# lucidrains/vector-quantize-pytorch

Measured on NVIDIA H100. Metric: vectors quantized/sec at dim=256, codebook=1024; indices bit-exact vs ref, higher is better.
Workload: dtype bf16

## Files before the change

### include/vqb200.h

```cpp
#ifndef VQB200_H
#define VQB200_H

#include <stddef.h>
#include <stdint.h>

#ifdef __cplusplus
extern "C" {
#endif

#define VQB_VERSION 100

#define VQB_DTYPE_F32 0
#define VQB_DTYPE_BF16 1

#define VQB_METRIC_EUCLID 0
#define VQB_METRIC_COSINE 1

#define VQB_OK 0
#define VQB_E_INVALID -1
#define VQB_E_UNSUPPORTED -2
#define VQB_E_ALIGN -3
#define VQB_E_NO_DEVICE -4
#define VQB_E_DRIVER -5
#define VQB_E_WORKSPACE -6
// ... 18 lines not shown
  void* resid_out;
  void* qsum;
  float* stats_cnt;
  float* stats_sum;
  int dtype;
  void* planes_out;
} vqb_fused_outputs;

int vqb_version(void);
const char* vqb_strerror(int code);

int vqb_padded_codes(int K);

int vqb_codebook_prepare(const float* embed, int K, int D, int metric, void* planes, void* bext, float* bias,
                         float* cnorm2, float* cmax, void* stream);

int vqb_input_prepare(const void* x, int dtype, int64_t N, int D, int metric, void* x_eff, void* a_planes,
                      int n_planes, void* stream);

int vqb_assign(const void* a_planes, int n_a, int64_t N, int D, const void* b_planes, const void* bext,
               const float* cmax, int K, float margin_rel, int n_passes, int32_t* idx, vqb_flag_entry* flagged,
               int32_t* flag_count, float* dbg_best, const vqb_fused_outputs* fused , void* stream);

int vqb_assign_ex(const void* a_planes, int n_a, int64_t N, int D, const void* b_planes, const void* bext,
                  const float* cmax, int K, float margin_rel, int n_passes, int32_t* idx, vqb_flag_entry* flagged,
                  int32_t* flag_count, float* dbg_best, const vqb_fused_outputs* fused, int metric, const float* cnorm2,
                  void* stream);

int vqb_debug_set_profile_buffer(void* device_buffer);
int vqb_debug_active(void);
int vqb_debug_set_mode(int mode);
int vqb_debug_graph_stats(long long* out4);
int vqb_debug_assign_plan(int n_a, int D, int n_passes, int* out6);
int vqb_debug_stats_plan(int64_t N, int K, int sms, int* out3);

int vqb_fix_flagged(const void* x_eff, int dtype, int64_t N, int D, const float* embed, const float* cnorm2, int K,
                    int metric, vqb_flag_entry* flagged, const int32_t* flag_count, int32_t* idx,
                    const vqb_fused_outputs* fused , void* stream);

int vqb_gather(const void* x_eff, int dtype, int64_t N, int D, const float* embed, const int32_t* idx, void* q_out,
               int64_t* idx64_out, int64_t idx_stride, double* loss_sum, const void* x_raw, void* resid_out, void* qsum,
               void* stream);

int vqb_loss_finalize(const double* loss_sum, int64_t numel, int dtype, float weight, float* loss_out, void* stream);

int64_t vqb_stats_offset(int K);
int64_t vqb_stats_floats(int K, int D);
size_t vqb_ema_stats_workspace(int64_t N, int K);
int vqb_ema_stats(const void* x_eff, int dtype, int64_t N, int D, const int32_t* idx, int K, float* stats,
                  void* workspace, size_t workspace_bytes, void* stream);

int vqb_ema_apply(float* cluster_size, float* embed_avg, float* embed, const float* stats, int K, int D, double decay,
                  double eps, int metric, int do_lerp, int do_normalise, void* planes, void* bext, float* bias,
                  float* cnorm2, float* cmax, float* scratch, void* stream);

int vqb_ema_apply_weighted(float* cluster_size, float* embed_avg, float* embed, const float* stats, int K, int D,
                           double decay, double eps, int metric, int do_lerp, int do_normalise, const float* code_weight,
                           void* planes, void* bext, float* bias, float* cnorm2, float* cmax, float* scratch, void* stream);

int vqb_peer_barrier(void* const* peer_flags_host, int rank, int world, uint32_t* epoch_dev, void* stream);
int vqb_ema_apply_peers(float* cluster_size, float* embed_avg, float* embed, const void* const* peer_stats_host, int world,
                        int64_t slice_offset, int K, int D, double decay, double eps, int metric, int do_normalise,
                        const float* code_weight, void* planes, void* bext, float* bias, float* cnorm2, float* cmax,
                        float* scratch, void* stream);

typedef struct vqb_vq_forward_args {
// ... 125 lines not shown
```

### vector_quantize_pytorch_b200/_C.py

```python
import ctypes
import os

from . import build as _build

_c = ctypes
_i32, _i64, _f32, _f64, _vp, _sz = _c.c_int, _c.c_int64, _c.c_float, _c.c_double, _c.c_void_p, _c.c_size_t

DTYPE_F32, DTYPE_BF16 = 0, 1
METRIC_EUCLID, METRIC_COSINE = 0, 1

class FusedOutputs(ctypes.Structure):
    _fields_ = [("x_eff", _vp), ("embed", _vp), ("q_out", _vp), ("idx64_out", _vp), ("idx_stride", _i64),
                ("loss_sum", _vp), ("x_raw", _vp), ("resid_out", _vp), ("qsum", _vp), ("stats_cnt", _vp), ("stats_sum", _vp),
                ("dtype", _i32), ("planes_out", _vp)]


class VQForwardArgs(ctypes.Structure):
    _fields_ = [("x", _vp), ("dtype", _i32), ("metric", _i32), ("N", _i64), ("D", _i32), ("K", _i32),
                ("already_normalised", _i32), ("cluster_size", _vp), ("embed_avg", _vp), ("embed", _vp),
                ("planes", _vp), ("bext", _vp), ("bias", _vp), ("cnorm2", _vp), ("cmax", _vp), ("scratch", _vp),
                ("q_out", _vp), ("idx64_out", _vp), ("idx_stride", _i64), ("loss_out", _vp), ("loss_weight", _f32),
                ("resid_out", _vp), ("qsum", _vp), ("idx32", _vp), ("update", _i32), ("stats_mode", _i32), ("stats_accumulate", _i32), ("do_normalise", _i32),
                ("decay", _f64), ("eps", _f64), ("stats", _vp), ("margin_rel", _f32), ("workspace", _vp),
                ("workspace_bytes", _sz), ("ev_search_begin", _vp), ("ev_search_end", _vp),
# ... 35 lines not shown
                ("bar", RvqBarArgs), ("emap", RvqEmaPeersArgs), ("simvq", RvqSimvqArgs)]


RVQ_STAGE, RVQ_EMA, RVQ_ACCUMULATE, RVQ_BARRIER, RVQ_EMA_PEERS, RVQ_SIMVQ_TAIL = 0, 1, 2, 3, 4, 5

SIGNATURES = {
    "vqb_version": (_i32, []),
    "vqb_strerror": (_c.c_char_p, [_i32]),
    "vqb_padded_codes": (_i32, [_i32]),
    "vqb_codebook_prepare": (_i32, [_vp, _i32, _i32, _i32, _vp, _vp, _vp, _vp, _vp, _vp]),
    "vqb_input_prepare": (_i32, [_vp, _i32, _i64, _i32, _i32, _vp, _vp, _i32, _vp]),
    "vqb_assign": (_i32, [_vp, _i32, _i64, _i32, _vp, _vp, _vp, _i32, _f32, _i32, _vp, _vp, _vp, _vp, _vp, _vp]),
    "vqb_assign_ex": (_i32, [_vp, _i32, _i64, _i32, _vp, _vp, _vp, _i32, _f32, _i32, _vp, _vp, _vp, _vp, _vp, _i32, _vp, _vp]),
    "vqb_fix_flagged": (_i32, [_vp, _i32, _i64, _i32, _vp, _vp, _i32, _i32, _vp, _vp, _vp, _vp, _vp]),
    "vqb_gather": (_i32, [_vp, _i32, _i64, _i32, _vp, _vp, _vp, _vp, _i64, _vp, _vp, _vp, _vp, _vp]),
    "vqb_loss_finalize": (_i32, [_vp, _i64, _i32, _f32, _vp, _vp]),
    "vqb_stats_offset": (_i64, [_i32]),
    "vqb_stats_floats": (_i64, [_i32, _i32]),
    "vqb_ema_stats_workspace": (_sz, [_i64, _i32]),
    "vqb_ema_stats": (_i32, [_vp, _i32, _i64, _i32, _vp, _i32, _vp, _vp, _sz, _vp]),
    "vqb_ema_apply": (_i32, [_vp, _vp, _vp, _vp, _i32, _i32, _f64, _f64, _i32, _i32, _i32, _vp, _vp, _vp, _vp, _vp, _vp, _vp]),
    "vqb_rotate": (_i32, [_vp, _vp, _vp, _i64, _i32, _i32, _vp, _vp]),
    "vqb_diveq": (_i32, [_vp, _vp, _vp, _vp, _i64, _i32, _i32, _f32, _vp, _vp, _vp]),
    "vqb_peer_barrier": (_i32, [_vp, _i32, _i32, _vp, _vp]),
    "vqb_ema_apply_peers": (_i32, [_vp, _vp, _vp, _vp, _i32, _i64, _i32, _i32, _f64, _f64, _i32, _i32, _vp, _vp, _vp, _vp, _vp, _vp, _vp, _vp]),
    "vqb_ema_apply_weighted": (_i32, [_vp, _vp, _vp, _vp, _i32, _i32, _f64, _f64, _i32, _i32, _i32, _vp, _vp, _vp, _vp, _vp, _vp, _vp, _vp]),
    "vqb_vq_forward_workspace": (_sz, [_i64, _i32, _i32, _i32, _i32, _i32]),
    "vqb_vq_forward": (_i32, [_vp, _vp]),
    "vqb_debug_set_profile_buffer": (_i32, [_vp]),
    "vqb_debug_set_mode": (_i32, [_i32]),
    "vqb_debug_active": (_i32, []),
    "vqb_debug_graph_stats": (_i32, [_vp]),
    "vqb_debug_assign_plan": (_i32, [_i32, _i32, _i32, _vp]),
    "vqb_debug_stats_plan": (_i32, [_i64, _i32, _i32, _vp]),
    "vqb_decode": (_i32, [_vp, _i64, _i32, _i32, _i32, _vp, _i64, _vp, _i32, _vp]),
    "vqb_rvq_accumulate": (_i32, [_vp, _i64, _i32, _i32, _i32, _vp, _i64, _vp, _i32, _vp]),
    "vqb_debug_gather_sum_plan": (_i32, [_i32, _i32, _i32, _i32, _i64, _i32, _vp]),
    "vqb_rvq_forward": (_i32, [_vp, _i32, _vp]),
    "vqb_rsimvq_tail": (_i32, [_vp, _vp, _vp, _i64, _i32, _i32, _vp, _vp, _i32, _vp, _i64, _vp, _vp, _f32, _f32, _vp]),
    "vqb_rsimvq_backward": (_i32, [_vp, _vp, _i32, _i32, _vp, _i64, _i32, _i32, _i32, _vp, _vp, _vp, _vp]),
    "vqb_fsq_forward": (_i32, [_vp, _i32, _i32, _i64, _i32, _i32, _i32, _i32, _i32, _i32, _vp, _vp, _vp, _vp, _vp, _i32, _i64, _i64,
                               _i64, _vp]),
    "vqb_fsq_backward": (_i32, [_vp, _i32, _i32, _i64, _i32, _i32, _i32, _i32, _i32, _i32, _vp, _vp, _vp, _vp, _vp, _vp]),
    "vqb_fsq_decode": (_i32, [_vp, _i32, _i64, _i64, _i64, _i64, _i32, _i32, _i32, _i32, _i32, _vp, _vp, _vp, _vp, _vp, _vp]),
    "vqb_lfq_forward": (_i32, [_vp, _i32, _i64, _i32, _i32, _i32, _i32, _i32, _i32, _i32, _vp, _vp, _vp, _i64, _i64, _i64, _vp, _vp,
                               _vp, _i32, _vp]),
    "vqb_lfq_forward_blocks": (_i32, [_i64, _i32]),
    "vqb_lfq_entropy": (_i32, [_vp, _i64, _i32, _i32, _i32, _vp, _i64, _i64, _vp, _f32, _i32, _vp, _vp, _vp]),
    "vqb_lfq_entropy_tiles": (_i32, [_i32]),
    "vqb_lfq_entropy_backward": (_i32, [_vp, _i64, _i32, _i32, _i32, _vp, _i64, _i64, _vp, _f32, _vp, _vp, _i32, _vp, _vp, _vp]),
    "vqb_lfq_backward": (_i32, [_vp, _i32, _i64, _i32, _i32, _i32, _i32, _i32, _i32, _i32, _vp, _vp, _vp, _vp, _vp, _vp, _vp]),
    "vqb_lfq_decode": (_i32, [_vp, _i32, _i64, _i64, _i64, _i64, _i32, _i32, _i32, _vp, _vp, _vp, _vp]),
    "vqb_fsp_blocks": (_i32, [_i64]),
    "vqb_fsp_forward": (_i32, [_vp, _i32, _i64, _i32, _i32, _i32, _vp, _f32, _vp, _vp, _f32, _f32, _f32, _vp, _vp, _vp, _vp, _i32,
                               _vp]),
    "vqb_fsp_stats": (_i32, [_vp, _i32, _i64, _i32, _vp, _vp, _i32, _vp, _vp, _vp, _vp]),
    "vqb_fsp_backward": (_i32, [_vp, _i32, _i64, _i32, _i32, _i32, _vp, _i32, _vp, _vp, _vp, _vp, _vp, _vp]),
    "vqb_fsp_decode": (_i32, [_vp, _i32, _i64, _i32, _i32, _i32, _vp, _f32, _f32, _vp, _vp, _vp]),
    "vqb_binmap_hot": (_i32, [_vp, _vp, _i64, _i32, _vp, _vp]),
    "vqb_binmap_backward_plan": (_i32, [_i64, _i32, _i32, _vp]),
    "vqb_binmap_backward": (_i32, [_vp, _i64, _i32, _vp, _i64, _i64, _i32, _vp, _vp, _vp]),
}


def _load():
    path = os.environ.get("VQB200_LIB")
# ... 27 lines not shown
```

### vector_quantize_pytorch_b200/csrc/ptx.cuh

```cuda
#pragma once
#include <cuda.h>
#include <cuda_runtime.h>
#include <stdint.h>

namespace vqb {

__device__ __forceinline__ uint32_t smem_u32(const void* p) {
  return static_cast<uint32_t>(__cvta_generic_to_shared(p));
}

__device__ __forceinline__ void mbar_init(uint32_t bar, uint32_t count) {
  asm volatile("mbarrier.init.shared::cta.b64 [%0], %1;" ::"r"(bar), "r"(count));
}
__device__ __forceinline__ void fence_barrier_init() {
  asm volatile("fence.mbarrier_init.release.cluster;" ::: "memory");
}
__device__ __forceinline__ void mbar_arrive(uint32_t bar) {
  asm volatile("mbarrier.arrive.shared::cta.b64 _, [%0];" ::"r"(bar) : "memory");
}
__device__ __forceinline__ void mbar_arrive_expect_tx(uint32_t bar, uint32_t bytes) {
  asm volatile("mbarrier.arrive.expect_tx.shared::cta.b64 _, [%0], %1;" ::"r"(bar), "r"(bytes) : "memory");
}
__device__ __forceinline__ bool mbar_try_wait(uint32_t bar, uint32_t parity) {
  uint32_t ok;
  asm volatile(
      "{\n"
      ".reg .pred p;\n"
      "mbarrier.try_wait.parity.shared::cta.b64 p, [%1], %2;\n"
      "selp.u32 %0, 1, 0, p;\n"
      "}\n"
      : "=r"(ok)
      : "r"(bar), "r"(parity)
      : "memory");
  return ok != 0;
}

#ifndef VQB_WAIT_TIMEOUT_CYCLES
#define VQB_WAIT_TIMEOUT_CYCLES (8000000000ll)
#endif
__device__ __forceinline__ void mbar_wait(uint32_t bar, uint32_t parity) {
  if (mbar_try_wait(bar, parity)) return;
  const long long t0 = clock64();
  while (!mbar_try_wait(bar, parity)) {
    if (clock64() - t0 > VQB_WAIT_TIMEOUT_CYCLES) __trap();
  }
}

__device__ __forceinline__ void tma_prefetch_desc(const CUtensorMap* m) {
  asm volatile("prefetch.tensormap [%0];" ::"l"(reinterpret_cast<uint64_t>(m)) : "memory");
}
__device__ __forceinline__ void tma_load_3d(uint32_t dst, const CUtensorMap* m, uint32_t bar, int c0, int c1, int c2) {
  asm volatile(
      "cp.async.bulk.tensor.3d.shared::cluster.global.tile.mbarrier::complete_tx::bytes [%0], [%1, {%3, %4, %5}], [%2];"
      ::"r"(dst), "l"(reinterpret_cast<uint64_t>(m)), "r"(bar), "r"(c0), "r"(c1), "r"(c2)
      : "memory");
}

__device__ __forceinline__ void tma_prefetch_l2_3d(const CUtensorMap* m, int c0, int c1, int c2) {
  asm volatile("cp.async.bulk.prefetch.tensor.3d.L2.global.tile [%0, {%1, %2, %3}];"
               ::"l"(reinterpret_cast<uint64_t>(m)), "r"(c0), "r"(c1), "r"(c2)
               : "memory");
}

__device__ __forceinline__ uint64_t wgmma_desc_sw128(uint32_t saddr) {
  uint64_t d = 0;
  d |= static_cast<uint64_t>((saddr >> 4) & 0x3FFF);
  d |= static_cast<uint64_t>(1) << 16;
  d |= static_cast<uint64_t>(1024 >> 4) << 32;
  d |= static_cast<uint64_t>(1) << 62;
  return d;
}

__device__ __forceinline__ uint64_t wgmma_desc_sw32(uint32_t saddr) {
  uint64_t d = 0;
  d |= static_cast<uint64_t>((saddr >> 4) & 0x3FFF);
  d |= static_cast<uint64_t>(1) << 16;
  d |= static_cast<uint64_t>(256 >> 4) << 32;
  d |= static_cast<uint64_t>(3) << 62;
  return d;
}

__device__ __forceinline__ void fence_proxy_async_shared() { asm volatile("fence.proxy.async.shared::cta;" ::: "memory"); }
__device__ __forceinline__ void wgmma_fence() { asm volatile("wgmma.fence.sync.aligned;" ::: "memory"); }
__device__ __forceinline__ void wgmma_commit() { asm volatile("wgmma.commit_group.sync.aligned;" ::: "memory"); }
template <int N>
__device__ __forceinline__ void wgmma_wait() { asm volatile("wgmma.wait_group.sync.aligned %0;" ::"n"(N) : "memory"); }

// ... 158 lines not shown
```

### vector_quantize_pytorch_b200/csrc/vq_assign.cu

```cuda
#include <type_traits>
#include "ptx.cuh"
#include "vqb_common.cuh"
#include "gather_row.cuh"
#include "epilogue.cuh"

#ifdef VQB_PROFILE
#define PROF_CLOCK() clock64()
#else
#define PROF_CLOCK() 0ll
#endif

namespace vqb {

constexpr int BM = 128;
constexpr int WM = 64;
constexpr int BN_STAGE = 128;
constexpr int BK = 64;
constexpr int A_SUB_BYTES = BM * BK * 2;
constexpr int B_SUB_BYTES = BN_STAGE * BK * 2;
constexpr int MAX_A_SUB = 8;
constexpr int MAX_STAGES = 8;
constexpr int NUM_CONSUMER_WARPS = 8;
constexpr int NUM_STORE_WARPS = 3;
constexpr int NUM_THREADS = 128 + NUM_CONSUMER_WARPS * 32;
constexpr int SMEM_CTRL_BYTES = 14336;
constexpr int SMEM_LIMIT = 232448;
constexpr int SEED_BYTES = BN_STAGE * 32;

struct AssignParams {
  int64_t N;
  int D, K, Kpad;
  int n_a, n_passes;
  int KB;
  int n_stages;
  int n_seed;
  int stream_a;
  const uint16_t* a_global;
  const uint16_t* bext;
  int num_row_tiles, num_code_steps;
  float margin_rel;
  const float* cmax;
  int32_t* idx;
  int32_t* idx_prov;
  int32_t* hist;
  int hist_shift;
  vqb_flag_entry* flagged;
  int32_t* flag_count;
  float* dbg_best;
  const uint8_t* row_mask;
  long long* prof;
  FusedOut fo;
  int copy_mode;
  int resid_mode;
  int metric;
  const uint16_t* b_hi;
  const float* cnorm2;
  uint32_t tagmask, mul1, mulm1;
// ... 54 lines not shown

template <int TAIL, int WN>
__global__ void __launch_bounds__(NUM_THREADS, 1)
vq_assign_kernel(const __grid_constant__ CUtensorMap tmA, const __grid_constant__ CUtensorMap tmB,
                 const __grid_constant__ CUtensorMap tmS, const AssignParams p) {
  static_assert(WN == 128 || WN == 256, "code step width");
  constexpr int SPAN = WN / BN_STAGE;
  constexpr uint32_t STEP_SEED_BYTES = SPAN * SEED_BYTES;
  extern __shared__ __align__(1024) uint8_t smem[];
  Ctrl* ctrl = reinterpret_cast<Ctrl*>(smem);
  const uint32_t smem_base = smem_u32(smem);
  const uint32_t a_base = (smem_base + SMEM_CTRL_BYTES + 1023u) & ~1023u;
  const bool stream_a = WN == 128 && p.stream_a;
  const int n_sub = stream_a ? 0 : p.n_a * p.KB;
  const uint32_t b_base = a_base + n_sub * A_SUB_BYTES;
  const uint32_t a_stage_bytes = stream_a ? A_SUB_BYTES : 0;
  const uint32_t stage_stride = a_stage_bytes + SPAN * B_SUB_BYTES;
  const int n_ring = p.n_stages / SPAN;
  const uint32_t seed_base = b_base + n_ring * stage_stride;

  const int warp = threadIdx.x >> 5;
  const int lane = threadIdx.x & 31;

  if (threadIdx.x == 0) {
    tma_prefetch_desc(&tmA);
    tma_prefetch_desc(&tmB);
    tma_prefetch_desc(&tmS);
    for (int s = 0; s < n_sub; ++s) {
      mbar_init(smem_u32(&ctrl->a_full[s]), 1);
      mbar_init(smem_u32(&ctrl->a_empty[s]), NUM_CONSUMER_WARPS);
    }
    for (int s = 0; s < n_ring; ++s) {
      mbar_init(smem_u32(&ctrl->b_full[s]), 1);
      mbar_init(smem_u32(&ctrl->b_empty[s]), NUM_CONSUMER_WARPS);
    }
    for (int s = 0; s < 2; ++s) {
      mbar_init(smem_u32(&ctrl->g_full[s]), NUM_CONSUMER_WARPS);
      mbar_init(smem_u32(&ctrl->g_empty[s]), NUM_STORE_WARPS);
    }
    fence_barrier_init();
  }
  if constexpr (WN == 256) {
    for (int i = threadIdx.x; i < WM * 16 / 2; i += NUM_THREADS) StepLocals<256>::bias_ones()[i] = 0x3F803F80u;
    fence_proxy_async_shared();
  }
  __syncthreads();

  if (warp == 0) {
    if (lane == 0) {
      long long w_empty = 0, w_aempty = 0;
      const long long pstart = PROF_CLOCK();
      int stage = 0, gstep = 0;
      uint32_t ph = 0;
      for (int t = 0, tile = static_cast<int>(blockIdx.x); tile < p.num_row_tiles; ++t, tile += static_cast<int>(gridDim.x)) {
        const int row0 = tile * BM;
        if (!stream_a && tile + static_cast<int>(gridDim.x) < p.num_row_tiles) {
          for (int ap = 0; ap < p.n_a; ++ap)
            for (int kb = 0; kb < p.KB; ++kb) tma_prefetch_l2_3d(&tmA, kb * BK, row0 + static_cast<int>(gridDim.x) * BM, ap);
        }
        for (int ct = 0; ct < p.num_code_steps; ++ct, ++gstep) {
          for (int kb = 0; kb < p.KB; ++kb) {
            for (int ps = 0; ps < p.n_passes; ++ps) {
              const int bplane = (ps == 1) ? 1 : 0;
              const int aplane = (ps == 2) ? 1 : 0;
              if (!stream_a && ct == 0 && (ps == 0 || ps == 2)) {
                const int sub = aplane * p.KB + kb;
                { const long long c0 = PROF_CLOCK(); mbar_wait(smem_u32(&ctrl->a_empty[sub]), (t & 1) ^ 1); w_aempty += PROF_CLOCK() - c0; }
                mbar_arrive_expect_tx(smem_u32(&ctrl->a_full[sub]), A_SUB_BYTES);
                tma_load_3d(a_base + sub * A_SUB_BYTES, &tmA, smem_u32(&ctrl->a_full[sub]), kb * BK, row0, aplane);
              }
              { const long long c0 = PROF_CLOCK(); mbar_wait(smem_u32(&ctrl->b_empty[stage]), ph ^ 1); w_empty += PROF_CLOCK() - c0; }
              const bool seeds = kb == 0 && ps == 0;
              mbar_arrive_expect_tx(smem_u32(&ctrl->b_full[stage]), stage_stride + (seeds ? STEP_SEED_BYTES : 0));
              if (seeds)
                tma_load_3d(seed_base + (gstep % p.n_seed) * STEP_SEED_BYTES, &tmS, smem_u32(&ctrl->b_full[stage]), 0, ct * WN, 0);
              if (stream_a)
                tma_load_3d(b_base + stage * stage_stride, &tmA, smem_u32(&ctrl->b_full[stage]), kb * BK, row0, aplane);
              tma_load_3d(b_base + stage * stage_stride + a_stage_bytes, &tmB, smem_u32(&ctrl->b_full[stage]), kb * BK,
                          ct * WN, bplane);
              if (++stage == n_ring) { stage = 0; ph ^= 1; }
            }
          }
        }
      }
      if (p.prof) {
        p.prof[blockIdx.x * 16 + 0] = w_empty;
        p.prof[blockIdx.x * 16 + 1] = PROF_CLOCK() - pstart;
        p.prof[blockIdx.x * 16 + 6] = w_aempty;
      }
    }
  } else if (warp <= NUM_STORE_WARPS) {
    const int sw = warp - 1;
    float lsum = 0.f;
    for (int t = 0, tile = static_cast<int>(blockIdx.x); p.fo.enabled && tile < p.num_row_tiles; ++t, tile += static_cast<int>(gridDim.x)) {
      mbar_wait(smem_u32(&ctrl->g_full[t & 1]), (t >> 1) & 1);
      const int* gi = ctrl->gidx[t & 1];
      if (TAIL >= 1) {
        constexpr int CB = 4;
        const bool bf = p.fo.dtype == VQB_DTYPE_BF16;
        const int row_bytes = p.D * (bf ? 2 : 4);
        const uint8_t* src = bf ? reinterpret_cast<const uint8_t*>(p.b_hi) : reinterpret_cast<const uint8_t*>(p.fo.embed);
        const uint8_t* xin = static_cast<const uint8_t*>(p.fo.x_eff);
        uint8_t* dst = static_cast<uint8_t*>(TAIL == 2 ? p.fo.resid_out : p.fo.q_out);
        for (int r0 = sw * CB; r0 < BM; r0 += NUM_STORE_WARPS * CB) {
          int ks[CB];
          bool ex[CB];
#pragma unroll
          for (int b = 0; b < CB; ++b) {
            const int g = gi[r0 + b];
            ex[b] = g < -1;
            ks[b] = ex[b] ? -2 - g : g;
          }
          const int64_t row_base = static_cast<int64_t>(tile) * BM + r0;
          if (p.fo.idx64_out && lane < CB && ks[lane & (CB - 1)] >= 0) {
            int kk = 0;
#pragma unroll
            for (int b = 0; b < CB; ++b) kk = (lane == b) ? ks[b] : kk;
            p.fo.idx64_out[(row_base + lane) * p.fo.idx_stride] = kk;
          }
          if (dst || (ex[0] | ex[1] | ex[2] | ex[3])) {
            for (int off = lane * 16; off < row_bytes; off += 512) {
              uint4 v[CB];
#pragma unroll
              for (int b = 0; b < CB; ++b)
                if (ks[b] >= 0) v[b] = __ldg(reinterpret_cast<const uint4*>(src + static_cast<int64_t>(ks[b]) * row_bytes + off));
              if (TAIL == 1) {
#pragma unroll
// ... 43 lines not shown
          bool any = false;
#pragma unroll
          for (int b = 0; b < GB; ++b) {
            ks[b] = gi[r0 + b];
            rows[b] = ks[b] >= 0 ? static_cast<int64_t>(tile) * BM + r0 + b : -1;
            any |= ks[b] >= 0;
          }
          if (!any) continue;
          lsum += tail_rows<GB>(p.fo, rows, ks, p.D, lane);
        }
      }
      __syncwarp();
      if (lane == 0) mbar_arrive(smem_u32(&ctrl->g_empty[t & 1]));
    }
    if (p.fo.enabled && p.fo.loss_sum) {
      const double w = warp_sum(static_cast<double>(lsum));
      if (lane == 0) atomicAdd(p.fo.loss_sum, w);
    }
  } else {
    const int wg = (warp >> 2) - 1;
    const int q = lane & 3;
    const int rit0 = wg * WM + (warp & 3) * 16 + (lane >> 2);
    const int n_items = p.KB * p.n_passes;
    const uint32_t a_row_off = wg * WM * 128;
    const uint32_t bias_a = q == 0 ? 0x3F803F80u : (q == 1 ? 0x00003F80u : 0u);
    long long w_full = 0, w_afull = 0, w_gap = 0, gap0 = -1;
    const long long cstart = PROF_CLOCK();
    float acc[WN / 2];
    int stage = 0, gstep = 0;
    uint32_t ph = 0;
    StepLocals<WN> locals;
    auto release = [&](int st, int sub) {
      if (lane == 0) {
        mbar_arrive(smem_u32(&ctrl->b_empty[st]));
        if (sub >= 0) mbar_arrive(smem_u32(&ctrl->a_empty[sub]));
      }
    };
    auto row_norms = [&](int tile, float (&xlo)[2]) {
#pragma unroll
      for (int h = 0; h < 2; ++h) {
        const int64_t row = static_cast<int64_t>(tile) * BM + rit0 + 8 * h;
        float a = 0.f, alo = 0.f;
        if (row < p.N) {
          const uint16_t* hp = p.a_global + row * p.D;
          for (int c = q * 8; c < p.D; c += 32) {
            const uint4 u = __ldg(reinterpret_cast<const uint4*>(hp + c));
            uint4 l = make_uint4(0u, 0u, 0u, 0u);
            if (p.n_a == 2) l = __ldg(reinterpret_cast<const uint4*>(hp + p.N * p.D + c));
            const uint32_t w[4] = {u.x, u.y, u.z, u.w};
            const uint32_t wl[4] = {l.x, l.y, l.z, l.w};
#pragma unroll
            for (int e = 0; e < 4; ++e) {
              const float h0 = __uint_as_float(w[e] << 16), h1 = __uint_as_float(w[e] & 0xFFFF0000u);
              const float l0 = __uint_as_float(wl[e] << 16), l1 = __uint_as_float(wl[e] & 0xFFFF0000u);
              a = fmaf(h0 + l0, h0 + l0, a);
              a = fmaf(h1 + l1, h1 + l1, a);
              alo = fmaf(l0, l0, alo);
              alo = fmaf(l1, l1, alo);
            }
          }
        }
        a += __shfl_xor_sync(0xffffffffu, a, 1);
        a += __shfl_xor_sync(0xffffffffu, a, 2);
        alo += __shfl_xor_sync(0xffffffffu, alo, 1);
        alo += __shfl_xor_sync(0xffffffffu, alo, 2);
        if (q == 0) ctrl->x2[rit0 + 8 * h] = a;
        xlo[h] = alo;
      }
    };
    auto init_band = [&](auto (&sc)[2], float (&xlo)[2]) {
      const bool euclid = p.metric != VQB_METRIC_COSINE;
      const float cmax = __ldg(p.cmax + CMAX_NORM);
      const float cres = __ldg(p.cmax + CMAX_RES);
      const float caux = p.n_a == 2 ? 0x1.02p-8f * cmax + __ldg(p.cmax + CMAX_LO) : 0.f;
      __syncwarp();
#pragma unroll
      for (int h = 0; h < 2; ++h) {
        const float x2 = ctrl->x2[rit0 + 8 * h];
        const float xn = sqrtf(x2);
        const float xc = xn * cmax;
        xlo[h] = p.n_a == 2 ? sqrtf(xlo[h]) * 1.0001f : 0.f;
        sc[h].init(2.f * (xn * cres + xlo[h] * caux + p.margin_rel * xc + (euclid ? 0x1p-21f * cmax * cmax : 0.f)) +
                   0x1p-18f * (xc + (euclid ? 0.5f * cmax * cmax : 0.f)) +
                   (euclid ? 0x1p-22f * (x2 + cmax * cmax) + 1e-8f : 1e-30f));
      }
    };
    for (int t = 0, tile = static_cast<int>(blockIdx.x); tile < p.num_row_tiles; ++t, tile += static_cast<int>(gridDim.x)) {
      typename std::conditional<WN == 128, ScanReg, ScanState<16>>::type sc[2];
      ScanQueue<16> sq[2];

      float xlo[2] = {0.f, 0.f};
      for (int ct = 0; ct < p.num_code_steps; ++ct) {
        const bool last_ct = ct == p.num_code_steps - 1;
        if (WN == 256 && ct == 0) {
          row_norms(tile, xlo);
          init_band(sc, xlo);
        }
        if (gap0 >= 0) w_gap += PROF_CLOCK() - gap0;
        { const long long c0 = PROF_CLOCK(); mbar_wait(smem_u32(&ctrl->b_full[stage]), ph); w_full += PROF_CLOCK() - c0; }
        wgmma_fence();
        const uint64_t sd = wgmma_desc_sw32(seed_base + (gstep % p.n_seed) * STEP_SEED_BYTES);
        if constexpr (WN == 128) wgmma_m64n128k16_bf16_rs_set(acc, bias_a, sd);
        else wgmma_m64n256k16_bf16_ss_set(acc, wgmma_desc_sw32(smem_u32(StepLocals<256>::bias_ones())), sd);
        int kb = 0, ps = 0;
        int pend_stage = -1, pend_sub = -1;
        for (int i = 0; i < n_items; ++i) {
          const int aplane = (ps == 2) ? 1 : 0;
          const int sub = aplane * p.KB + kb;
          if (ct == 0 && !stream_a) { const long long c0 = PROF_CLOCK(); mbar_wait(smem_u32(&ctrl->a_full[sub]), t & 1); w_afull += PROF_CLOCK() - c0; }
          if (i > 0) { const long long c0 = PROF_CLOCK(); mbar_wait(smem_u32(&ctrl->b_full[stage]), ph); w_full += PROF_CLOCK() - c0; }
          const uint32_t st_addr = b_base + stage * stage_stride;
          const uint32_t a_addr = (stream_a ? st_addr : a_base + sub * A_SUB_BYTES) + a_row_off;
          const uint64_t ad = wgmma_desc_sw128(a_addr);
          const uint64_t bd = wgmma_desc_sw128(st_addr + a_stage_bytes);
          fence_regs(acc);
          wgmma_fence();
#pragma unroll
          for (int k = 0; k < 8; k += 2) {
            if constexpr (WN == 128) wgmma_m64n128k16_bf16(acc, ad + k, bd + k);
            else wgmma_m64n256k16_bf16(acc, ad + k, bd + k);
// ... 76 lines not shown
            p.idx[row] = i0;
            if (p.idx_prov) p.idx_prov[row] = (n < 2) ? i0 : -1;
            if (p.hist && n < 2) atomicAdd(p.hist + static_cast<size_t>(tile >> p.hist_shift) * p.K + i0, 1);
            if (p.dbg_best) p.dbg_best[row] = best;
            if (n >= 2) {
              const bool many = n > 3;
              const int s = many ? static_cast<int>(p.N) - 1 - atomicAdd(p.flag_count + 1, 1) : atomicAdd(p.flag_count, 1);
              vqb_flag_entry e;
              e.row = static_cast<int32_t>(row);
              e.cand0 = many ? 0 : i0;
              e.cand1 = many ? 0 : i1;
              e.cand2 = rr.i2;
              e.count = n;
              e.pad[0] = e.pad[1] = e.pad[2] = 0;
              p.flagged[s] = e;
            }
          }
        }
        __syncwarp();
      }
      if (p.fo.enabled && lane == 0) mbar_arrive(smem_u32(&ctrl->g_full[t & 1]));
    }
    if (TAIL >= 1 && p.fo.loss_sum) {
      const double w = warp_sum(static_cast<double>(locals.loss()));
      if (lane == 0) atomicAdd(p.fo.loss_sum, w);
    }
    if (p.prof && threadIdx.x == 128) {
      p.prof[blockIdx.x * 16 + 2] = w_full;
      p.prof[blockIdx.x * 16 + 3] = PROF_CLOCK() - cstart;
      p.prof[blockIdx.x * 16 + 4] = w_gap;
      p.prof[blockIdx.x * 16 + 5] = w_afull;
    }
  }
}

typedef CUresult (*PFN_encodeTiled)(CUtensorMap*, CUtensorMapDataType, cuuint32_t, void*, const cuuint64_t*,
                                    const cuuint64_t*, const cuuint32_t*, const cuuint32_t*, CUtensorMapInterleave,
                                    CUtensorMapSwizzle, CUtensorMapL2promotion, CUtensorMapFloatOOBfill);

static PFN_encodeTiled get_encode_fn() {
  static PFN_encodeTiled fn = nullptr;
  static bool tried = false;
  if (!tried) {
    tried = true;
    void* f = nullptr;
    cudaDriverEntryPointQueryResult qres;
    if (cudaGetDriverEntryPoint("cuTensorMapEncodeTiled", &f, cudaEnableDefault, &qres) == cudaSuccess &&
        qres == cudaDriverEntryPointSuccess)
      fn = reinterpret_cast<PFN_encodeTiled>(f);
  }
  return fn;
}

static int make_map(CUtensorMap* m, const void* base, int cols, int64_t rows, int planes, int box_cols, int box_rows,
                    CUtensorMapSwizzle swz) {
  PFN_encodeTiled enc = get_encode_fn();
  if (!enc) return VQB_E_DRIVER;
  cuuint64_t dims[3] = {static_cast<cuuint64_t>(cols), static_cast<cuuint64_t>(rows), static_cast<cuuint64_t>(planes)};
  cuuint64_t strides[2] = {static_cast<cuuint64_t>(cols) * 2, static_cast<cuuint64_t>(cols) * 2 * static_cast<cuuint64_t>(rows)};
  cuuint32_t box[3] = {static_cast<cuuint32_t>(box_cols), static_cast<cuuint32_t>(box_rows), 1};
  cuuint32_t estr[3] = {1, 1, 1};
  CUresult r = enc(m, CU_TENSOR_MAP_DATA_TYPE_BFLOAT16, 3, const_cast<void*>(base), dims, strides, box, estr,
                   CU_TENSOR_MAP_INTERLEAVE_NONE, swz, CU_TENSOR_MAP_L2_PROMOTION_L2_256B, CU_TENSOR_MAP_FLOAT_OOB_FILL_NONE);
  return r == CUDA_SUCCESS ? VQB_OK : VQB_E_DRIVER;
}

// ... 6 lines not shown
  if (n_passes == 0) n_passes = n_a + 1;
  if (n_passes != n_a + 1) return VQB_E_UNSUPPORTED;
  if (D % 8 != 0) return VQB_E_UNSUPPORTED;
  const int KB = (D + BK - 1) / BK;
  const int stream_a = n_a * KB > MAX_A_SUB ? 1 : 0;
  const int a_bytes = stream_a ? 0 : n_a * KB * A_SUB_BYTES;
  const int stage_bytes = B_SUB_BYTES + (stream_a ? A_SUB_BYTES : 0);
  const int fixed = SMEM_CTRL_BYTES + 1024  + a_bytes;
  const int n_items = KB * n_passes;
  int stages = MAX_STAGES;
  auto seed_slots = [&](int st) { return (st + n_items - 1) / n_items; };
  while (stages >= 2 && fixed + stages * stage_bytes + seed_slots(stages) * SEED_BYTES > SMEM_LIMIT) --stages;
  if (stages < 2) return VQB_E_UNSUPPORTED;
  pl->stream_a = stream_a;
  pl->n_stages = stages;
  pl->n_seed = seed_slots(stages);
  pl->n_items = n_items;
  pl->KB = KB;
  pl->smem_bytes = fixed + stages * stage_bytes + pl->n_seed * SEED_BYTES;
  return VQB_OK;
}

static bool wide_step(const AssignPlan& pl, int Kpad, int* n_seed, int* smem_bytes) {
  if (pl.stream_a || pl.n_stages % 2 != 0 || Kpad <= BN_STAGE) return false;
  const int ring = pl.n_stages / 2;
  const int seeds = (ring + pl.n_items - 1) / pl.n_items;
  const int bytes = pl.smem_bytes - pl.n_seed * SEED_BYTES + seeds * 2 * SEED_BYTES;
  if (bytes + WIDE_STATIC_SMEM > SMEM_LIMIT) return false;
  *n_seed = seeds;
  *smem_bytes = bytes;
  return true;
}

}

using namespace vqb;

extern "C" int vqb_debug_assign_plan(int n_a, int D, int n_passes, int* out6) {
  if (!out6) return VQB_E_INVALID;
  AssignPlan pl;
  const int rc = assign_plan(n_a, D, n_passes, &pl);
  if (rc) return rc;
  out6[0] = pl.stream_a; out6[1] = pl.n_stages; out6[2] = pl.n_seed;
  out6[3] = pl.n_items; out6[4] = pl.KB; out6[5] = pl.smem_bytes;
  return VQB_OK;
}

extern "C" int vqb_padded_codes(int K) {
  if (K <= 0) return 0;
  const int BN = code_tile(K);
  return (K + BN - 1) / BN * BN;
}

static long long* g_prof = nullptr;
static int g_dbg_mode = 0;
extern "C" int vqb_debug_set_mode(int mode) { g_dbg_mode = mode; return VQB_OK; }
extern "C" int vqb_debug_active(void) { return (g_prof != nullptr) || (g_dbg_mode != 0); }
extern "C" int vqb_debug_set_profile_buffer(void* buf) { g_prof = static_cast<long long*>(buf); return VQB_OK; }

extern "C" int vqb_assign(const void* a_planes, int n_a, int64_t N, int D, const void* b_planes, const void* bext,
                          const float* cmax, int K, float margin_rel, int n_passes, int32_t* idx,
                          vqb_flag_entry* flagged, int32_t* flag_count, float* dbg_best,
                          const vqb_fused_outputs* fused, void* stream) {
  return vqb_assign_ex(a_planes, n_a, N, D, b_planes, bext, cmax, K, margin_rel, n_passes, idx, flagged, flag_count,
                       dbg_best, fused, VQB_METRIC_EUCLID, nullptr, stream);
}

extern "C" int vqb_assign_ex(const void* a_planes, int n_a, int64_t N, int D, const void* b_planes, const void* bext,
                             const float* cmax, int K, float margin_rel, int n_passes, int32_t* idx,
                             vqb_flag_entry* flagged, int32_t* flag_count, float* dbg_best,
                             const vqb_fused_outputs* fused, int metric, const float* cnorm2, void* stream) {
  return vqb::assign_launch(a_planes, n_a, N, D, b_planes, bext, cmax, K, margin_rel, n_passes, idx, nullptr, nullptr, 0,
                            flagged, flag_count, dbg_best, fused, metric, cnorm2, stream);
}

int vqb::assign_launch(const void* a_planes, int n_a, int64_t N, int D, const void* b_planes, const void* bext,
                       const float* cmax, int K, float margin_rel, int n_passes, int32_t* idx, int32_t* idx_prov,
                       int32_t* hist, int hist_shift, vqb_flag_entry* flagged, int32_t* flag_count, float* dbg_best,
                       const vqb_fused_outputs* fused, int metric, const float* cnorm2, void* stream, const uint8_t* row_mask) {
  if (!a_planes || !b_planes || !bext || !cmax || !idx || !flagged || !flag_count) return VQB_E_INVALID;
  if (N <= 0 || K <= 0) return VQB_E_INVALID;
  AssignPlan plan;
  int rc = assign_plan(n_a, D, n_passes, &plan);
  if (rc) return rc;
// ... 5 lines not shown
  rc = make_fused(&p.fo, fused, D, N);
  if (rc) return rc;
  rc = check_device();
  if (rc) return rc;

  p.N = N; p.D = D; p.K = K;
  p.Kpad = vqb_padded_codes(K);
  p.n_a = n_a; p.n_passes = n_passes; p.KB = plan.KB;
  p.num_row_tiles = static_cast<int>((N + BM - 1) / BM);
  int smem_bytes = plan.smem_bytes;
  p.n_seed = plan.n_seed;
  const bool wide = wide_step(plan, p.Kpad, &p.n_seed, &smem_bytes);
  const int WN = wide ? 256 : 128;
  p.num_code_steps = (p.Kpad + WN - 1) / WN;
  p.margin_rel = margin_rel;
  p.cmax = cmax; p.idx = idx; p.idx_prov = idx_prov; p.hist = hist; p.hist_shift = hist_shift; p.flagged = flagged; p.flag_count = flag_count; p.dbg_best = dbg_best;
  p.row_mask = row_mask;
  p.prof = g_prof;
  p.tagmask = 0xFFFFFFF0u; p.mul1 = 1u; p.mulm1 = 0xFFFFFFFFu;
  p.metric = metric;
  p.cnorm2 = cnorm2;
  p.b_hi = static_cast<const uint16_t*>(b_planes);
  p.bext = static_cast<const uint16_t*>(bext);
  p.copy_mode = p.fo.enabled && !p.fo.resid_out && !(metric == VQB_METRIC_COSINE && p.fo.loss_sum && !cnorm2);
  p.resid_mode = p.fo.enabled && p.fo.resid_out && !p.fo.q_out &&
                 (!p.fo.x_raw || p.fo.x_raw == p.fo.x_eff) && !(metric == VQB_METRIC_COSINE && p.fo.loss_sum && !cnorm2);
  p.stream_a = plan.stream_a;
  p.a_global = static_cast<const uint16_t*>(a_planes);
  p.n_stages = plan.n_stages;

  CUtensorMap tmA, tmB, tmS;
  rc = make_map(&tmA, a_planes, D, N, n_a, BK, BM, CU_TENSOR_MAP_SWIZZLE_128B);
  if (rc) return rc;
  rc = make_map(&tmB, b_planes, D, p.Kpad, 2, BK, WN, CU_TENSOR_MAP_SWIZZLE_128B);
  if (rc) return rc;
  rc = make_map(&tmS, bext, 16, p.Kpad, 1, 16, WN, CU_TENSOR_MAP_SWIZZLE_32B);
  if (rc) return rc;

  static bool attr_set = false;
  if (!attr_set) {
    void (*const kernels[6])(CUtensorMap, CUtensorMap, CUtensorMap, AssignParams) = {
        vq_assign_kernel<0, 128>, vq_assign_kernel<1, 128>, vq_assign_kernel<2, 128>,
        vq_assign_kernel<0, 256>, vq_assign_kernel<1, 256>, vq_assign_kernel<2, 256>};
    for (int i = 0; i < 6; ++i) {
      const int dyn = i < 3 ? SMEM_LIMIT : SMEM_LIMIT - WIDE_STATIC_SMEM;
      const cudaError_t e = cudaFuncSetAttribute(kernels[i], cudaFuncAttributeMaxDynamicSharedMemorySize, dyn);
      if (e != cudaSuccess) return static_cast<int>(e);
    }
    attr_set = true;
  }
  const int grid = p.num_row_tiles < num_sms() ? p.num_row_tiles : num_sms();
  cudaStream_t s = static_cast<cudaStream_t>(stream);
  if (wide) {
    if (p.copy_mode) vq_assign_kernel<1, 256><<<grid, NUM_THREADS, smem_bytes, s>>>(tmA, tmB, tmS, p);
    else if (p.resid_mode) vq_assign_kernel<2, 256><<<grid, NUM_THREADS, smem_bytes, s>>>(tmA, tmB, tmS, p);
    else vq_assign_kernel<0, 256><<<grid, NUM_THREADS, smem_bytes, s>>>(tmA, tmB, tmS, p);
  } else {
    if (p.copy_mode) vq_assign_kernel<1, 128><<<grid, NUM_THREADS, smem_bytes, s>>>(tmA, tmB, tmS, p);
    else if (p.resid_mode) vq_assign_kernel<2, 128><<<grid, NUM_THREADS, smem_bytes, s>>>(tmA, tmB, tmS, p);
    else vq_assign_kernel<0, 128><<<grid, NUM_THREADS, smem_bytes, s>>>(tmA, tmB, tmS, p);
  }
  return static_cast<int>(cudaGetLastError());
}
```

Before: 389.1 million.

## Launch assign kernel as 2-CTA clusters with TMA multicast of codebook tiles

Launches the assign kernel in clusters of two CTAs. Each CTA loads half of every codebook (B) and seed tile and multicasts it to both CTAs, roughly halving L2-to-SMEM codebook traffic per CTA. Empty barriers now count arrivals from both CTAs, and cluster syncs are added at start and end. The grid is sized from cluster occupancy. In exchange the two CTAs are lockstepped, the row-tile loop bound is changed, and the odd CTA of the last pair may process an out-of-range tile.

```diff
diff --git a/include/vqb200.h b/include/vqb200.h
--- a/include/vqb200.h
+++ b/include/vqb200.h
@@ -74,6 +74,7 @@
 int vqb_debug_set_mode(int mode);
 int vqb_debug_graph_stats(long long* out4);
 int vqb_debug_assign_plan(int n_a, int D, int n_passes, int* out6);
+int vqb_debug_assign_grid(int n_a, int D, int K, int64_t N, int* out2);
 int vqb_debug_stats_plan(int64_t N, int K, int sms, int* out3);
 
 int vqb_fix_flagged(const void* x_eff, int dtype, int64_t N, int D, const float* embed, const float* cnorm2, int K,
diff --git a/vector_quantize_pytorch_b200/_C.py b/vector_quantize_pytorch_b200/_C.py
--- a/vector_quantize_pytorch_b200/_C.py
+++ b/vector_quantize_pytorch_b200/_C.py
@@ -91,6 +91,7 @@
     "vqb_debug_active": (_i32, []),
     "vqb_debug_graph_stats": (_i32, [_vp]),
     "vqb_debug_assign_plan": (_i32, [_i32, _i32, _i32, _vp]),
+    "vqb_debug_assign_grid": (_i32, [_i32, _i32, _i32, _i64, _vp]),
     "vqb_debug_stats_plan": (_i32, [_i64, _i32, _i32, _vp]),
     "vqb_decode": (_i32, [_vp, _i64, _i32, _i32, _i32, _vp, _i64, _vp, _i32, _vp]),
     "vqb_rvq_accumulate": (_i32, [_vp, _i64, _i32, _i32, _i32, _vp, _i64, _vp, _i32, _vp]),
diff --git a/vector_quantize_pytorch_b200/csrc/ptx.cuh b/vector_quantize_pytorch_b200/csrc/ptx.cuh
--- a/vector_quantize_pytorch_b200/csrc/ptx.cuh
+++ b/vector_quantize_pytorch_b200/csrc/ptx.cuh
@@ -46,6 +46,26 @@
   }
 }
 
+__device__ __forceinline__ uint32_t cluster_ctarank() {
+  uint32_t r;
+  asm volatile("mov.u32 %0, %%cluster_ctarank;" : "=r"(r));
+  return r;
+}
+__device__ __forceinline__ void mbar_arrive_pair(uint32_t bar) {
+  asm volatile(
+      "{\n"
+      ".reg .b32 r0, r1;\n"
+      "mapa.shared::cluster.u32 r0, %0, 0;\n"
+      "mapa.shared::cluster.u32 r1, %0, 1;\n"
+      "mbarrier.arrive.shared::cluster.b64 _, [r0];\n"
+      "mbarrier.arrive.shared::cluster.b64 _, [r1];\n"
+      "}\n" ::"r"(bar) : "memory");
+}
+__device__ __forceinline__ void cluster_sync() {
+  asm volatile("barrier.cluster.arrive.release;\n"
+               "barrier.cluster.wait.acquire;" ::: "memory");
+}
+
 __device__ __forceinline__ void tma_prefetch_desc(const CUtensorMap* m) {
   asm volatile("prefetch.tensormap [%0];" ::"l"(reinterpret_cast<uint64_t>(m)) : "memory");
 }
@@ -53,6 +73,15 @@
   asm volatile(
       "cp.async.bulk.tensor.3d.shared::cluster.global.tile.mbarrier::complete_tx::bytes [%0], [%1, {%3, %4, %5}], [%2];"
       ::"r"(dst), "l"(reinterpret_cast<uint64_t>(m)), "r"(bar), "r"(c0), "r"(c1), "r"(c2)
+      : "memory");
+}
+
+__device__ __forceinline__ void tma_load_3d_mc(uint32_t dst, const CUtensorMap* m, uint32_t bar, int c0, int c1, int c2,
+                                               uint16_t cta_mask) {
+  asm volatile(
+      "cp.async.bulk.tensor.3d.shared::cluster.global.tile.mbarrier::complete_tx::bytes.multicast::cluster"
+      " [%0], [%1, {%3, %4, %5}], [%2], %6;"
+      ::"r"(dst), "l"(reinterpret_cast<uint64_t>(m)), "r"(bar), "r"(c0), "r"(c1), "r"(c2), "h"(cta_mask)
       : "memory");
 }
 
diff --git a/vector_quantize_pytorch_b200/csrc/vq_assign.cu b/vector_quantize_pytorch_b200/csrc/vq_assign.cu
--- a/vector_quantize_pytorch_b200/csrc/vq_assign.cu
+++ b/vector_quantize_pytorch_b200/csrc/vq_assign.cu
@@ -23,6 +23,7 @@
 constexpr int NUM_CONSUMER_WARPS = 8;
 constexpr int NUM_STORE_WARPS = 3;
 constexpr int NUM_THREADS = 128 + NUM_CONSUMER_WARPS * 32;
+constexpr int PAIR = 2;
 constexpr int SMEM_CTRL_BYTES = 14336;
 constexpr int SMEM_LIMIT = 232448;
 constexpr int SEED_BYTES = BN_STAGE * 32;
@@ -143,7 +144,7 @@
     }
     for (int s = 0; s < n_ring; ++s) {
       mbar_init(smem_u32(&ctrl->b_full[s]), 1);
-      mbar_init(smem_u32(&ctrl->b_empty[s]), NUM_CONSUMER_WARPS);
+      mbar_init(smem_u32(&ctrl->b_empty[s]), PAIR * NUM_CONSUMER_WARPS);
     }
     for (int s = 0; s < 2; ++s) {
       mbar_init(smem_u32(&ctrl->g_full[s]), NUM_CONSUMER_WARPS);
@@ -155,7 +156,7 @@
     for (int i = threadIdx.x; i < WM * 16 / 2; i += NUM_THREADS) StepLocals<256>::bias_ones()[i] = 0x3F803F80u;
     fence_proxy_async_shared();
   }
-  __syncthreads();
+  cluster_sync();
 
   if (warp == 0) {
     if (lane == 0) {
@@ -163,7 +164,7 @@
       const long long pstart = PROF_CLOCK();
       int stage = 0, gstep = 0;
       uint32_t ph = 0;
-      for (int t = 0, tile = static_cast<int>(blockIdx.x); tile < p.num_row_tiles; ++t, tile += static_cast<int>(gridDim.x)) {
+      for (int t = 0, tile = static_cast<int>(blockIdx.x); (tile & ~1) < p.num_row_tiles; ++t, tile += static_cast<int>(gridDim.x)) {
         const int row0 = tile * BM;
         if (!stream_a && tile + static_cast<int>(gridDim.x) < p.num_row_tiles) {
           for (int ap = 0; ap < p.n_a; ++ap)
@@ -182,13 +183,16 @@
               }
               { const long long c0 = PROF_CLOCK(); mbar_wait(smem_u32(&ctrl->b_empty[stage]), ph ^ 1); w_empty += PROF_CLOCK() - c0; }
               const bool seeds = kb == 0 && ps == 0;
-              mbar_arrive_expect_tx(smem_u32(&ctrl->b_full[stage]), stage_stride + (seeds ? STEP_SEED_BYTES : 0));
+              const uint32_t full = smem_u32(&ctrl->b_full[stage]);
+              const int rank = static_cast<int>(cluster_ctarank());
+              mbar_arrive_expect_tx(full, stage_stride + (seeds ? STEP_SEED_BYTES : 0));
               if (seeds)
-                tma_load_3d(seed_base + (gstep % p.n_seed) * STEP_SEED_BYTES, &tmS, smem_u32(&ctrl->b_full[stage]), 0, ct * WN, 0);
+                tma_load_3d_mc(seed_base + (gstep % p.n_seed) * STEP_SEED_BYTES + rank * (WN / 2) * 32, &tmS, full, 0,
+                               ct * WN + rank * (WN / 2), 0, 0x3);
               if (stream_a)
-                tma_load_3d(b_base + stage * stage_stride, &tmA, smem_u32(&ctrl->b_full[stage]), kb * BK, row0, aplane);
-              tma_load_3d(b_base + stage * stage_stride + a_stage_bytes, &tmB, smem_u32(&ctrl->b_full[stage]), kb * BK,
-                          ct * WN, bplane);
+                tma_load_3d(b_base + stage * stage_stride, &tmA, full, kb * BK, row0, aplane);
+              tma_load_3d_mc(b_base + stage * stage_stride + a_stage_bytes + rank * (WN / 2) * 128, &tmB, full, kb * BK,
+                             ct * WN + rank * (WN / 2), bplane, 0x3);
               if (++stage == n_ring) { stage = 0; ph ^= 1; }
             }
           }
@@ -203,7 +207,7 @@
   } else if (warp <= NUM_STORE_WARPS) {
     const int sw = warp - 1;
     float lsum = 0.f;
-    for (int t = 0, tile = static_cast<int>(blockIdx.x); p.fo.enabled && tile < p.num_row_tiles; ++t, tile += static_cast<int>(gridDim.x)) {
+    for (int t = 0, tile = static_cast<int>(blockIdx.x); p.fo.enabled && (tile & ~1) < p.num_row_tiles; ++t, tile += static_cast<int>(gridDim.x)) {
       mbar_wait(smem_u32(&ctrl->g_full[t & 1]), (t >> 1) & 1);
       const int* gi = ctrl->gidx[t & 1];
       if (TAIL >= 1) {
@@ -313,7 +317,7 @@
     StepLocals<WN> locals;
     auto release = [&](int st, int sub) {
       if (lane == 0) {
-        mbar_arrive(smem_u32(&ctrl->b_empty[st]));
+        mbar_arrive_pair(smem_u32(&ctrl->b_empty[st]));
         if (sub >= 0) mbar_arrive(smem_u32(&ctrl->a_empty[sub]));
       }
     };
@@ -366,7 +370,7 @@
                    (euclid ? 0x1p-22f * (x2 + cmax * cmax) + 1e-8f : 1e-30f));
       }
     };
-    for (int t = 0, tile = static_cast<int>(blockIdx.x); tile < p.num_row_tiles; ++t, tile += static_cast<int>(gridDim.x)) {
+    for (int t = 0, tile = static_cast<int>(blockIdx.x); (tile & ~1) < p.num_row_tiles; ++t, tile += static_cast<int>(gridDim.x)) {
       typename std::conditional<WN == 128, ScanReg, ScanState<16>>::type sc[2];
       ScanQueue<16> sq[2];
 
@@ -509,6 +513,7 @@
       p.prof[blockIdx.x * 16 + 5] = w_afull;
     }
   }
+  cluster_sync();
 }
 
 typedef CUresult (*PFN_encodeTiled)(CUtensorMap*, CUtensorMapDataType, cuuint32_t, void*, const cuuint64_t*,
@@ -581,6 +586,47 @@
   return true;
 }
 
+typedef void (*AssignKernel)(CUtensorMap, CUtensorMap, CUtensorMap, AssignParams);
+static const AssignKernel kAssignKernels[6] = {
+    vq_assign_kernel<0, 128>, vq_assign_kernel<1, 128>, vq_assign_kernel<2, 128>,
+    vq_assign_kernel<0, 256>, vq_assign_kernel<1, 256>, vq_assign_kernel<2, 256>};
+
+static int resident_pairs(int ki, int smem_bytes, int* pairs) {
+  static bool attr_set = false;
+  if (!attr_set) {
+    for (int i = 0; i < 6; ++i) {
+      const int dyn = i < 3 ? SMEM_LIMIT : SMEM_LIMIT - WIDE_STATIC_SMEM;
+      const cudaError_t e = cudaFuncSetAttribute(kAssignKernels[i], cudaFuncAttributeMaxDynamicSharedMemorySize, dyn);
+      if (e != cudaSuccess) return static_cast<int>(e);
+    }
+    attr_set = true;
+  }
+  static int c_dev[6] = {-1, -1, -1, -1, -1, -1}, c_smem[6], c_pairs[6];
+  int dev = 0;
+  if (cudaGetDevice(&dev) != cudaSuccess) return VQB_E_NO_DEVICE;
+  if (c_dev[ki] != dev || c_smem[ki] != smem_bytes) {
+    cudaLaunchConfig_t cfg = {};
+    cudaLaunchAttribute attr[1];
+    attr[0].id = cudaLaunchAttributeClusterDimension;
+    attr[0].val.clusterDim.x = PAIR;
+    attr[0].val.clusterDim.y = 1;
+    attr[0].val.clusterDim.z = 1;
+    cfg.gridDim = dim3(PAIR);
+    cfg.blockDim = dim3(NUM_THREADS);
+    cfg.dynamicSmemBytes = static_cast<size_t>(smem_bytes);
+    cfg.attrs = attr;
+    cfg.numAttrs = 1;
+    int n = 0;
+    const cudaError_t e = cudaOccupancyMaxActiveClusters(&n, kAssignKernels[ki], &cfg);
+    if (e != cudaSuccess) return static_cast<int>(e);
+    if (n < 1) return VQB_E_UNSUPPORTED;
+    const int half = num_sms() / PAIR;
+    c_dev[ki] = dev; c_smem[ki] = smem_bytes; c_pairs[ki] = n < half ? n : half;
+  }
+  *pairs = c_pairs[ki];
+  return VQB_OK;
+}
+
 }
 
 using namespace vqb;
@@ -599,6 +645,23 @@
   if (K <= 0) return 0;
   const int BN = code_tile(K);
   return (K + BN - 1) / BN * BN;
+}
+
+extern "C" int vqb_debug_assign_grid(int n_a, int D, int K, int64_t N, int* out2) {
+  if (!out2 || N <= 0 || K <= 0) return VQB_E_INVALID;
+  AssignPlan pl;
+  int rc = assign_plan(n_a, D, 0, &pl);
+  if (rc) return rc;
+  rc = check_device();
+  if (rc) return rc;
+  int n_seed = pl.n_seed, smem_bytes = pl.smem_bytes, pairs;
+  const bool wide = wide_step(pl, vqb_padded_codes(K), &n_seed, &smem_bytes);
+  rc = resident_pairs(wide ? 3 : 0, smem_bytes, &pairs);
+  if (rc) return rc;
+  const int64_t need = (N + 2 * BM - 1) / (2 * BM);
+  out2[0] = pairs;
+  out2[1] = PAIR * static_cast<int>(need < pairs ? need : pairs);
+  return VQB_OK;
 }
 
 static long long* g_prof = nullptr;
@@ -670,33 +733,28 @@
   CUtensorMap tmA, tmB, tmS;
   rc = make_map(&tmA, a_planes, D, N, n_a, BK, BM, CU_TENSOR_MAP_SWIZZLE_128B);
   if (rc) return rc;
-  rc = make_map(&tmB, b_planes, D, p.Kpad, 2, BK, WN, CU_TENSOR_MAP_SWIZZLE_128B);
-  if (rc) return rc;
-  rc = make_map(&tmS, bext, 16, p.Kpad, 1, 16, WN, CU_TENSOR_MAP_SWIZZLE_32B);
-  if (rc) return rc;
-
-  static bool attr_set = false;
-  if (!attr_set) {
-    void (*const kernels[6])(CUtensorMap, CUtensorMap, CUtensorMap, AssignParams) = {
-        vq_assign_kernel<0, 128>, vq_assign_kernel<1, 128>, vq_assign_kernel<2, 128>,
-        vq_assign_kernel<0, 256>, vq_assign_kernel<1, 256>, vq_assign_kernel<2, 256>};
-    for (int i = 0; i < 6; ++i) {
-      const int dyn = i < 3 ? SMEM_LIMIT : SMEM_LIMIT - WIDE_STATIC_SMEM;
-      const cudaError_t e = cudaFuncSetAttribute(kernels[i], cudaFuncAttributeMaxDynamicSharedMemorySize, dyn);
-      if (e != cudaSuccess) return static_cast<int>(e);
-    }
-    attr_set = true;
-  }
-  const int grid = p.num_row_tiles < num_sms() ? p.num_row_tiles : num_sms();
-  cudaStream_t s = static_cast<cudaStream_t>(stream);
-  if (wide) {
-    if (p.copy_mode) vq_assign_kernel<1, 256><<<grid, NUM_THREADS, smem_bytes, s>>>(tmA, tmB, tmS, p);
-    else if (p.resid_mode) vq_assign_kernel<2, 256><<<grid, NUM_THREADS, smem_bytes, s>>>(tmA, tmB, tmS, p);
-    else vq_assign_kernel<0, 256><<<grid, NUM_THREADS, smem_bytes, s>>>(tmA, tmB, tmS, p);
-  } else {
-    if (p.copy_mode) vq_assign_kernel<1, 128><<<grid, NUM_THREADS, smem_bytes, s>>>(tmA, tmB, tmS, p);
-    else if (p.resid_mode) vq_assign_kernel<2, 128><<<grid, NUM_THREADS, smem_bytes, s>>>(tmA, tmB, tmS, p);
-    else vq_assign_kernel<0, 128><<<grid, NUM_THREADS, smem_bytes, s>>>(tmA, tmB, tmS, p);
-  }
+  rc = make_map(&tmB, b_planes, D, p.Kpad, 2, BK, WN / PAIR, CU_TENSOR_MAP_SWIZZLE_128B);
+  if (rc) return rc;
+  rc = make_map(&tmS, bext, 16, p.Kpad, 1, 16, WN / PAIR, CU_TENSOR_MAP_SWIZZLE_32B);
+  if (rc) return rc;
+
+  const int ki = (wide ? 3 : 0) + (p.copy_mode ? 1 : (p.resid_mode ? 2 : 0));
+  int pairs = 0;
+  rc = resident_pairs(ki, smem_bytes, &pairs);
+  if (rc) return rc;
+  const int need = (p.num_row_tiles + PAIR - 1) / PAIR;
+  cudaLaunchConfig_t cfg = {};
+  cudaLaunchAttribute attr[1];
+  attr[0].id = cudaLaunchAttributeClusterDimension;
+  attr[0].val.clusterDim.x = PAIR;
+  attr[0].val.clusterDim.y = 1;
+  attr[0].val.clusterDim.z = 1;
+  cfg.gridDim = dim3(PAIR * (need < pairs ? need : pairs));
+  cfg.blockDim = dim3(NUM_THREADS);
+  cfg.dynamicSmemBytes = static_cast<size_t>(smem_bytes);
+  cfg.stream = static_cast<cudaStream_t>(stream);
+  cfg.attrs = attr;
+  cfg.numAttrs = 1;
+  cudaLaunchKernelEx(&cfg, kAssignKernels[ki], tmA, tmB, tmS, p);
   return static_cast<int>(cudaGetLastError());
 }
```

Result: no change. 386.4 million (median of 6 runs) (-0.7%).
